# microsoft/GenerativeImage2Text

Hardware: NVIDIA H100
Metric: captions/sec (greedy, max_len=40) GIT_BASE batch64 (higher is better)
Workload: dtype bf16

## Files before the change

generativeimage2text_b200/csrc/attention.cuh:

```cuda
#pragma once
#include "ptx.cuh"
#include "rowops.cuh"

namespace gitb200 {

struct AttnParams {
  const __nv_bfloat16* q;
  const __nv_bfloat16* k;
  const __nv_bfloat16* v;
  __nv_bfloat16* out;
  int B, S, H;
  long long q_rs, kv_rs, q_bs, kv_bs, o_rs, o_bs;
  float scale_log2;
  const int* seq_lens;
};

constexpr int kAttnWgRows = 64;
constexpr int kAttnWgSmem = 5 * 8192 + 64 + 1024;

template <class LoadKV, class Mask>
__device__ __forceinline__ void attn_wg_tile(const CUtensorMap* tmQ, int q_col, int q_row, int nblk, float scale_log2,
                                             const LoadKV& load_kv, const Mask& mask, float (&o)[32]) {
  extern __shared__ __align__(1024) uint8_t attn_smem_raw[];
  uint8_t* smem = attn_smem_raw + ((1024u - (smem_u32(attn_smem_raw) & 1023u)) & 1023u);
// ... 70 lines not shown
    __syncthreads();
    if (tid == 0 && blk + 2 < nblk) issue(blk + 2, st);
  }
#pragma unroll
  for (int i = 0; i < 2; ++i) {
    l_run[i] += __shfl_xor_sync(0xffffffffu, l_run[i], 1);
    l_run[i] += __shfl_xor_sync(0xffffffffu, l_run[i], 2);
  }
  const float inv0 = 1.0f / l_run[0], inv1 = 1.0f / l_run[1];
#pragma unroll
  for (int j = 0; j < 8; ++j) {
    o[4 * j] *= inv0;
    o[4 * j + 1] *= inv0;
    o[4 * j + 2] *= inv1;
    o[4 * j + 3] *= inv1;
  }
}

template <bool kRagged>
__global__ void __launch_bounds__(128) flash_attn_wgmma_kernel(const __grid_constant__ CUtensorMap tmQ,
                                                              const __grid_constant__ CUtensorMap tmK,
                                                              const __grid_constant__ CUtensorMap tmV, const AttnParams p) {
  const int tid = threadIdx.x, warp = tid >> 5, lane = tid & 31;
  const int h = blockIdx.y, b = blockIdx.z;
  const int S = kRagged ? p.seq_lens[b] : p.S;
  const int q0 = blockIdx.x * kAttnWgRows;
  const int row_base = b * p.S;
  if (kRagged && q0 >= S) {
    __nv_bfloat16* og = p.out + b * p.o_bs + h * 64;
    for (int i = tid; i < kAttnWgRows * 8; i += 128) {
      const int r = q0 + (i >> 3);
      if (r < p.S) *reinterpret_cast<uint4*>(og + static_cast<long long>(r) * p.o_rs + (i & 7) * 8) = make_uint4(0, 0, 0, 0);
    }
    return;
  }
  if (tid == 0) {
    tma_prefetch_desc(&tmQ);
    tma_prefetch_desc(&tmK);
    tma_prefetch_desc(&tmV);
  }
  auto load_kv = [&](int blk, uint8_t* sK, uint8_t* sV, uint64_t* bar) {
    tma_load_2d(sK, &tmK, bar, h * 64, row_base + blk * kAttnWgRows);
    tma_load_2d(sV, &tmV, bar, h * 64, row_base + blk * kAttnWgRows);
  };
  auto mask = [&](int blk, float (&s)[32]) {
    const int key0 = blk * kAttnWgRows + 2 * (lane & 3);
#pragma unroll
    for (int j = 0; j < 8; ++j) {
      const int key = key0 + 8 * j;
      if (key >= S) { s[4 * j] = -INFINITY; s[4 * j + 2] = -INFINITY; }
      if (key + 1 >= S) { s[4 * j + 1] = -INFINITY; s[4 * j + 3] = -INFINITY; }
    }
  };
  float o[32];
  attn_wg_tile(&tmQ, h * 64, row_base + q0, (S + kAttnWgRows - 1) / kAttnWgRows, p.scale_log2, load_kv, mask, o);
  const int r0 = q0 + warp * 16 + (lane >> 2), r1 = r0 + 8;
  __nv_bfloat16* og = p.out + b * p.o_bs + h * 64 + 2 * (lane & 3);
#pragma unroll
  for (int j = 0; j < 8; ++j) {
    if (r0 < S) *reinterpret_cast<uint32_t*>(og + static_cast<long long>(r0) * p.o_rs + 8 * j) = pack_bf16(o[4 * j], o[4 * j + 1]);
    else if (kRagged && r0 < p.S) *reinterpret_cast<uint32_t*>(og + static_cast<long long>(r0) * p.o_rs + 8 * j) = 0u;
    if (r1 < S) *reinterpret_cast<uint32_t*>(og + static_cast<long long>(r1) * p.o_rs + 8 * j) = pack_bf16(o[4 * j + 2], o[4 * j + 3]);
// ... 470 lines not shown
      mx = fmaxf(mx, a);
    }
  }
  mx = warp_max(mx);
  float sum = 0.f;
  for (int j = lane; j < n_keys; j += 32) {
    const float e = expf(sc[j] - mx);
    sc[j] = e;
    sum += e;
  }
  sum = warp_sum(sum);
  __syncwarp();
  float a0 = 0.f, a1 = 0.f;
  for (int j = 0; j < n_keys; ++j) {
    const float2 vv = *reinterpret_cast<const float2*>(key_row(j, true) + 2 * lane);
    a0 = fmaf(sc[j], vv.x, a0);
    a1 = fmaf(sc[j], vv.y, a1);
  }
  return make_float2(a0 / sum, a1 / sum);
}

__global__ void __launch_bounds__(128) attn_f32_kernel(const AttnF32Params p) {
  extern __shared__ __align__(16) float attn_f32_smem[];
  const int warp = threadIdx.x >> 5, lane = threadIdx.x & 31;
  float* q_s = attn_f32_smem + warp * (64 + p.S);
  const long long item = static_cast<long long>(blockIdx.x) * 4 + warp;
  const long long total = static_cast<long long>(p.B) * p.H * p.S;
  if (item >= total) return;
  const int row = static_cast<int>(item % p.S);
  const int h = static_cast<int>((item / p.S) % p.H);
  const int b = static_cast<int>(item / (static_cast<long long>(p.S) * p.H));
  const int S = p.seq_lens != nullptr ? p.seq_lens[b] : p.S;
  __nv_bfloat16* orow = p.out + b * p.o_bs + static_cast<long long>(row) * 3 * p.d_model;
  if (row >= S) {
    store_split3_pair(orow, p.d_model, h * 64 + 2 * lane, 0.f, 0.f);
    return;
  }
  const float* qg = p.q + b * p.q_bs + static_cast<long long>(row) * p.q_rs + h * 64;
  q_s[lane] = qg[lane] * 0.125f;
  q_s[lane + 32] = qg[lane + 32] * 0.125f;
  __syncwarp();
  const float2 r = attn_row_f32(q_s, q_s + 64, S, [&](int j, bool want_v) {
    return (want_v ? p.v : p.k) + b * p.kv_bs + static_cast<long long>(j) * p.kv_rs + h * 64;
  });
  store_split3_pair(orow, p.d_model, h * 64 + 2 * lane, r.x, r.y);
}
// ... 99 lines not shown
```

generativeimage2text_b200/csrc/engine_api.inc:

```

extern "C" int gitb200_encode(gitb200_engine* h, const float* images_dev, int batch, int frames, float* feats_out_dev,
                              void* stream) {
  if (!h) return 1;
  const gitb200_engine::NextCall in = take_next_call(h, false);
  ImageBatch ib;
  TRY(image_batch(h, "encode", batch, frames, in.image_hw, &ib));
  if (!images_dev) return fail(h, "encode: null images");
  cudaSetDevice(h->device);
  return encode_impl(h, images_dev, ib, feats_out_dev, static_cast<cudaStream_t>(stream));
}

static int init_src_rows(gitb200_engine* h, cudaStream_t st) {
  const int n = h->cur_rows * h->T_alloc;
  init_src_row_kernel<<<(n + 255) / 256, 256, 0, st>>>(h->src_row[0].as<int>(), h->cur_rows, h->T_alloc);
  CKL(h, "init_src_row_kernel");
  init_src_row_kernel<<<(n + 255) / 256, 256, 0, st>>>(h->src_row[1].as<int>(), h->cur_rows, h->T_alloc);
  CKL(h, "init_src_row_kernel");
  h->cur_src = 0;
  return 0;
}

extern "C" int gitb200_prefill(gitb200_engine* h, int batch, int beam, float* vproj_out_dev, void* stream) {
  if (!h) return 1;
  cudaSetDevice(h->device);
// ... 711 lines not shown
      dst = part_ws.p;
    }
    c = gemm_skinny(static_cast<const bf16*>(a_dev), K, static_cast<const bf16*>(w_dev), K, M, N, K, bias_dev, act, dst, N,
                    out_bf16 != 0, splits, nullptr);
  }
  c.bn = bn;
  int rc = launch_gemm(h, c, st);
  if (rc == 0 && splits > 1) {
    const long long n = static_cast<long long>(M) * N;
    sum_partials_kernel<<<static_cast<int>(std::min<long long>((n + 255) / 256, static_cast<long long>(h->num_sms) * 8)), 256, 0, st>>>(
        part_ws.as<float>(), static_cast<float*>(out_dev), n, c.p.k_splits);
    if (cudaGetLastError() != cudaSuccess) rc = fail(h, "op_gemm: sum_partials_kernel launch failed");
  }
  if (rc != 0) g_create_error = h->err;
  return rc;
}

extern "C" int gitb200_op_layernorm(const float* x_dev, const float* bias_dev, const float* resid_dev,
                                    const float* gamma_dev, const float* beta_dev, float eps, float* out_f32_dev,
                                    void* out_bf16_dev, int rows, int D, void* stream) {
  gitb200_engine* h = op_engine();
  if (!h) return fail(nullptr, "op_layernorm: no CUDA device");
  int rc = launch_ln(h, ln_params(x_dev, bias_dev, resid_dev, gamma_dev, beta_dev, eps, out_f32_dev,
                                  static_cast<bf16*>(out_bf16_dev), rows), D, static_cast<cudaStream_t>(stream));
  if (rc != 0) g_create_error = h->err;
  return rc;
}

static int op_gemm_ex_impl(gitb200_engine* h, const gitb200_gemm_desc& d, int* k_splits_out, cudaStream_t st) {
  if (!d.a || !d.b || !d.out[0]) return fail(h, "op_gemm_ex: null operand or output");
  if (d.M < 1 || d.N < 1 || d.K < 1) return fail(h, "op_gemm_ex: bad shape M=%d N=%d K=%d", d.M, d.N, d.K);
  if (d.act < ACT_NONE || d.act > ACT_QUICKGELU_EXACT) return fail(h, "op_gemm_ex: act %d outside 0 .. 3", d.act);
  if (d.k_splits < 1) return fail(h, "op_gemm_ex: k_splits %d < 1", d.k_splits);
  if (d.split3 && !d.out_bf16) return fail(h, "op_gemm_ex: split3 is a bf16 output format");
  if (d.transposed && (d.resid || d.lse_target || d.seg_n > 0 || d.rows_per_batch > 0))
    return fail(h, "op_gemm_ex: the transposed epilogue has no residual, statistics, column segments or row map");
  if (d.lse_target && (!d.bias || d.resid || d.act || d.out_bf16 || d.seg_n > 0 || d.rows_per_batch > 0 || d.k_splits > 1))
    return fail(h, "op_gemm_ex: the statistics epilogue takes a bias and nothing else");
  if (d.resid && d.ld_resid < d.N) return fail(h, "op_gemm_ex: ld_resid %lld < N", static_cast<long long>(d.ld_resid));
  const int seg_n = d.seg_n > 0 ? d.seg_n : d.N;
  if (d.N % seg_n != 0 || d.N / seg_n > 3) return fail(h, "op_gemm_ex: N=%d is not one to three segments of %d", d.N, seg_n);
  for (int s = 0; s < d.N / seg_n; ++s)
    if (!d.out[s]) return fail(h, "op_gemm_ex: output segment %d is null", s);
  const long long row_elems = d.lse_target ? 2LL * ((d.N + 255) / 256) : (d.transposed ? d.M : seg_n) * (d.split3 ? 3LL : 1LL);
  if (d.ldo < row_elems) return fail(h, "op_gemm_ex: ldo %lld < %lld", static_cast<long long>(d.ldo), row_elems);
  if (d.rows_per_batch > 0 && (d.batch_stride < d.rows_per_batch || d.row_offset < 0 ||
                               d.row_offset + d.rows_per_batch > d.batch_stride))
// ... 15 lines not shown
  return launch_gemm(h, c, st);
}

extern "C" int gitb200_op_gemm_ex(const gitb200_gemm_desc* desc, int* k_splits_out, void* stream) {
  gitb200_engine* h = op_engine();
  if (!h) return fail(nullptr, "op_gemm_ex: no CUDA device");
  const int rc = desc ? op_gemm_ex_impl(h, *desc, k_splits_out, static_cast<cudaStream_t>(stream))
                      : fail(h, "op_gemm_ex: null descriptor");
  if (rc != 0) g_create_error = h->err;
  return rc;
}

static int op_layernorm_ex_impl(gitb200_engine* h, LnParams p, int D, int pre, cudaStream_t st) {
  if (!p.x || !p.gamma || !p.beta) return fail(h, "op_layernorm_ex: null input");
  if (p.rows < 1) return fail(h, "op_layernorm_ex: rows %d < 1", p.rows);
  if (p.n_partials < 1) return fail(h, "op_layernorm_ex: n_partials %d < 1", p.n_partials);
  if (p.n_partials > 1 && p.partial_stride < static_cast<long long>(p.rows) * D)
    return fail(h, "op_layernorm_ex: partial_stride smaller than one partial buffer");
  if (p.split3 && !p.out_bf16) return fail(h, "op_layernorm_ex: split3 is a bf16 output format");
  if (p.remap_F < 0 || (p.remap_F > 0 && (p.remap_B < 1 || p.remap_L < 1 || p.rows != p.remap_B * p.remap_F * p.remap_L)))
    return fail(h, "op_layernorm_ex: %d rows are not B=%d x F=%d x L=%d", p.rows, p.remap_B, p.remap_F, p.remap_L);
  if (p.temb && p.remap_F == 0) return fail(h, "op_layernorm_ex: a temporal embedding needs the frame remap");
  if (pre && D != 768) return fail(h, "op_layernorm_ex: the PRE instantiation exists for D = 768 only");
  return launch_ln(h, p, D, st, pre != 0);
}

extern "C" int gitb200_op_layernorm_ex(const float* x_dev, int n_partials, long long partial_stride, const float* bias_dev,
                                       const float* resid_dev, const float* gamma_dev, const float* beta_dev, float eps,
                                       float* out_f32_dev, void* out_bf16_dev, int rows, int D, int split3,
                                       const float* temb_dev, int remap_B, int remap_F, int remap_L,
                                       const int32_t* skip_flag_dev, int pre, void* stream) {
  gitb200_engine* h = op_engine();
  if (!h) return fail(nullptr, "op_layernorm_ex: no CUDA device");
  LnParams p = ln_params(x_dev, bias_dev, resid_dev, gamma_dev, beta_dev, eps, out_f32_dev, static_cast<bf16*>(out_bf16_dev), rows);
  p.n_partials = n_partials; p.partial_stride = partial_stride;
  p.split3 = split3 ? 1 : 0;
  p.temb = temb_dev; p.remap_B = remap_B; p.remap_F = remap_F; p.remap_L = remap_L;
  p.skip_flag = skip_flag_dev;
  const int rc = op_layernorm_ex_impl(h, p, D, pre, static_cast<cudaStream_t>(stream));
  if (rc != 0) g_create_error = h->err;
  return rc;
}

static int op_lse_combine_impl(gitb200_engine* h, const void* parts, int n_parts, int rows, int T, int V, const int32_t* targets,
                               const int64_t* need_predict, float eps, float* logprob, float* row_loss, int32_t* row_valid,
                               float* loss, cudaStream_t st) {
  if (!parts || !targets || !need_predict || !logprob || !row_loss || !row_valid) return fail(h, "op_lse_combine: null buffer");
// ... 276 lines not shown
```

generativeimage2text_b200/csrc/gemm.cuh:

```cuda
#pragma once
#include "ptx.cuh"

namespace gitb200 {

struct GemmParams {
  int M, N, K;
  int k_splits;
  int transposed;
  int partial;
  long long split_stride;
  int act;
  int out_bf16;
  const float* bias;
  const float* resid;
  long long ld_resid;
  void* out[3];
  long long ldo;
  long long batch_stride;
  int seg_n;
  int rows_per_batch;
  int row_offset;
  const int* skip;
  unsigned long long* dbg;
  int split3;
// ... 245 lines not shown
  const int warp = (threadIdx.x >> 5) & 3;
  const int lane = threadIdx.x & 31;

  if (threadIdx.x == 0) {
    tma_prefetch_desc(&tmA);
    tma_prefetch_desc(&tmB);
    for (int s = 0; s < C::STAGES; ++s) {
      mbar_init(&full[s], 1);
      mbar_init(&empty[s], C::MMA_WGS);
    }
    mbar_fence_init();
  }
  __syncthreads();

  const int m_tiles = (p.M + C::BM - 1) / C::BM;
  const int n_tiles = (p.N + BN - 1) / BN;
  const int kb_total = (p.K + C::BK - 1) / C::BK;
  const int kb_per = (kb_total + p.k_splits - 1) / p.k_splits;
  const int mn_tiles = m_tiles * n_tiles;
  const int num_tiles = mn_tiles * p.k_splits;

  const bool chained = p.chain.counters != nullptr;
  int npre = 0;
  if (kTransposed && p.pdl && static_cast<int>(blockIdx.x) < num_tiles) {
    const int split = static_cast<int>(blockIdx.x) / mn_tiles;
    const int kb0 = split * kb_per;
    npre = min(C::STAGES, min(kb_total, kb0 + kb_per) - kb0);
    if (threadIdx.x == 0) {
      const int m_blk = (static_cast<int>(blockIdx.x) - split * mn_tiles) / n_tiles;
      for (int i = 0; i < npre; ++i) {
        mbar_arrive_expect_tx(&full[i], C::STAGE_BYTES);
        tma_load_2d(sA + i * C::A_BYTES, &tmA, &full[i], (kb0 + i) * C::BK, m_blk * C::BM);
      }
    }
  }
  if (chained) chain_wait(p.chain);
  else if (p.pdl) griddep_wait();
  if (p.pdl) tl_mark(1000 + static_cast<int>(gridDim.x));

  if (wg == 0) {
    setmaxnreg_dec<C::PRODUCER_REGS>();
    if (threadIdx.x == 0) {
      int stage = 0;
      uint32_t phase = 0;
      for (int tile = blockIdx.x; tile < num_tiles; tile += gridDim.x) {
        const int split = tile / mn_tiles;
        const int rem = tile - split * mn_tiles;
        const int m_blk = rem / n_tiles;
        const int n_blk = rem - m_blk * n_tiles;
        const int kb0 = split * kb_per;
        const int kb1 = min(kb_total, kb0 + kb_per);
        for (int kb = kb0; kb < kb1; ++kb) {
          if (npre > 0) {
            --npre;
            tma_load_2d(sB + stage * C::B_BYTES, &tmB, &full[stage], kb * C::BK, n_blk * BN);
          } else {
            mbar_wait(&empty[stage], phase ^ 1);
            mbar_arrive_expect_tx(&full[stage], C::STAGE_BYTES);
            tma_load_2d(sA + stage * C::A_BYTES, &tmA, &full[stage], kb * C::BK, m_blk * C::BM);
            tma_load_2d(sB + stage * C::B_BYTES, &tmB, &full[stage], kb * C::BK, n_blk * BN);
          }
          if (++stage == C::STAGES) {
            stage = 0;
            phase ^= 1;
          }
        }
      }
    }
  } else {
    setmaxnreg_inc<C::MMA_REGS>();
    const int mw = wg - 1;
    const bool store_ok = !(p.pdl && !chained && p.skip != nullptr && *p.skip != 0);
    uint8_t* stg_wg = sStage + mw * C::WG_STAGING_BYTES;
    uint8_t* stg = stg_wg + warp * (32 * 128);
    const int rsub = lane >> 3;
    float acc[BN / 2];
    int stage = 0;
    uint32_t phase = 0;
// ... 108 lines not shown
```

generativeimage2text_b200/csrc/gitb200.cu:

```cuda
#include <cuda.h>
#include <cuda_bf16.h>
#include <cuda_runtime.h>

#include <algorithm>
#include <atomic>
#include <cmath>
#include <cstdarg>
#include <cstdio>
#include <cstring>
#include <map>
#include <mutex>
#include <set>
#include <string>
#include <utility>
#include <vector>

#include "../../include/gitb200.h"
#include "attention.cuh"
#include "constrained.cuh"
#include "decode_mega.cuh"
#include "gemm.cuh"
#include "preproc.cuh"
#include "ptx.cuh"
#include "rowops.cuh"
// ... 376 lines not shown
    case 192: return launch_gemm_bn<192>(h, c, st);
    case 256: return launch_gemm_bn<256>(h, c, st);
    default: return fail(h, "gemm: unsupported tile width %d", bn);
  }
}

static GemmCall gemm_plain(const bf16* A, long long lda, const bf16* W, long long ldw, int M, int N, int K,
                           const float* bias, int act, const float* resid, void* out, bool out_bf16) {
  GemmCall c;
  c.A = A; c.lda = lda; c.B = W; c.ldb = ldw;
  c.p.M = M; c.p.N = N; c.p.K = K; c.p.k_splits = 1;
  c.p.bias = bias; c.p.act = act; c.p.resid = resid; c.p.ld_resid = N;
  c.p.out[0] = out; c.p.ldo = N; c.p.out_bf16 = out_bf16 ? 1 : 0;
  c.p.seg_n = N;
  return c;
}
enum class RowOut { F32, OPERAND, QKV };
static GemmCall gemm_rows(const gitb200_engine* h, RowOut kind, const bf16* A, const bf16* W, int M, int N, int K,
                          const float* bias, int act, const float* resid, void* out) {
  const int ks = h->ks();
  const bool bf16_out = kind == RowOut::OPERAND || (kind == RowOut::QKV && !h->parity);
  GemmCall c = gemm_plain(A, static_cast<long long>(K) * ks, W, static_cast<long long>(K) * ks, M, N, K * ks, bias,
                          (h->parity && act == ACT_QUICKGELU) ? ACT_QUICKGELU_EXACT : act, resid, out, bf16_out);
  if (kind == RowOut::OPERAND && h->parity) {
    c.p.split3 = 1;
    c.p.ldo = 3LL * N;
  }
  return c;
}
static GemmCall gemm_skinny(const bf16* X, long long ldx, const bf16* W, long long ldw, int rows, int feats, int K,
                            const float* bias, int act, void* out, long long ldo, bool out_bf16, int k_splits,
                            const int* skip, bool pdl = false) {
  GemmCall c;
  c.A = W; c.lda = ldw; c.B = X; c.ldb = ldx;
  c.p.M = feats; c.p.N = rows; c.p.K = K; c.p.k_splits = k_splits;
  c.p.transposed = 1; c.p.partial = k_splits > 1 ? 1 : 0;
  c.p.split_stride = static_cast<long long>(rows) * ldo;
  c.p.bias = bias; c.p.act = act;
  c.p.out[0] = out; c.p.ldo = ldo; c.p.out_bf16 = out_bf16 ? 1 : 0;
  c.p.skip = skip;
  c.p.pdl = pdl ? 1 : 0;
  return c;
}

static int launch_ln(gitb200_engine* h, const LnParams& p, int D, cudaStream_t st, bool pdl = false) {
  const int grid = (p.rows + 7) / 8;
  if (D == 768 && pdl) CK(launch_k(true, layernorm_kernel<768, true>, dim3(grid), dim3(256), 0, st, p));
  else if (D == 768) CK(launch_k(false, layernorm_kernel<768, false>, dim3(grid), dim3(256), 0, st, p));
  else if (D == 1024) CK(launch_k(pdl, layernorm_kernel<1024, false>, dim3(grid), dim3(256), 0, st, p));
  else return fail(h, "layernorm: unsupported width %d", D);
  CKL(h, "layernorm_kernel");
  return 0;
}
static LnParams ln_params(const float* x, const float* bias, const float* resid, const float* g, const float* b,
                          float eps, float* of32, bf16* obf16, int rows) {
  LnParams p{};
  p.x = x; p.bias = bias; p.resid = resid; p.gamma = g; p.beta = b; p.eps = eps;
  p.out_f32 = of32; p.out_bf16 = obf16; p.rows = rows;
  return p;
}
static LnParams ln_operand(const gitb200_engine* h, const float* x, const float* g, const float* b, float eps, float* of32,
                           bf16* obf16, int rows) {
  LnParams p = ln_params(x, nullptr, nullptr, g, b, eps, of32, obf16, rows);
  p.split3 = h->parity ? 1 : 0;
  return p;
}

struct SelfAttn {
  const void* q;
  const void* k;
  const void* v;
  bf16* out;
  int B, S, H;
  long long q_rs, kv_rs, q_bs, kv_bs, o_rs, o_bs;
  const int* seq_lens;
};
static int launch_self_attention(gitb200_engine* h, const SelfAttn& a, bool fp32, cudaStream_t st) {
  if (fp32) {
    AttnF32Params p{};
    p.q = static_cast<const float*>(a.q); p.k = static_cast<const float*>(a.k); p.v = static_cast<const float*>(a.v);
    p.out = a.out;
    p.B = a.B; p.S = a.S; p.H = a.H; p.d_model = a.H * 64;
    p.q_rs = a.q_rs; p.kv_rs = a.kv_rs; p.q_bs = a.q_bs; p.kv_bs = a.kv_bs; p.o_bs = a.o_bs;
    p.seq_lens = a.seq_lens;
    const size_t smem = static_cast<size_t>(4) * (64 + p.S) * sizeof(float);
    if (smem > 200 * 1024) return fail(h, "parity attention: %d keys do not fit in shared memory", p.S);
    TRY(set_dyn_smem(h, reinterpret_cast<const void*>(attn_f32_kernel), smem));
    const long long items = static_cast<long long>(p.B) * p.H * p.S;
    attn_f32_kernel<<<static_cast<unsigned int>((items + 3) / 4), 128, smem, st>>>(p);
    CKL(h, "attn_f32_kernel");
    return 0;
  }
  if (a.q_bs != static_cast<long long>(a.S) * a.q_rs || a.kv_bs != static_cast<long long>(a.S) * a.kv_rs)
    return fail(h, "attention: batches must be stored back to back (batch stride = S * row stride)");
  AttnParams p{};
  p.q = static_cast<const bf16*>(a.q); p.k = static_cast<const bf16*>(a.k); p.v = static_cast<const bf16*>(a.v);
  p.out = a.out;
  p.B = a.B; p.S = a.S; p.H = a.H;
  p.q_rs = a.q_rs; p.kv_rs = a.kv_rs; p.q_bs = a.q_bs; p.kv_bs = a.kv_bs; p.o_rs = a.o_rs; p.o_bs = a.o_bs;
  p.scale_log2 = 0.125f * 1.44269504088896340736f;
  p.seq_lens = a.seq_lens;
  const long long rows = static_cast<long long>(a.B) * a.S;
  CUtensorMap tq, tk, tv;
  TRY(get_tmap(h, a.q, rows, a.H * 64, a.q_rs, kAttnWgRows, &tq));
  TRY(get_tmap(h, a.k, rows, a.H * 64, a.kv_rs, kAttnWgRows, &tk));
  TRY(get_tmap(h, a.v, rows, a.H * 64, a.kv_rs, kAttnWgRows, &tv));
  const dim3 grid((a.S + kAttnWgRows - 1) / kAttnWgRows, a.H, a.B);
  if (a.seq_lens != nullptr) flash_attn_wgmma_kernel<true><<<grid, 128, kAttnWgSmem, st>>>(tq, tk, tv, p);
  else flash_attn_wgmma_kernel<false><<<grid, 128, kAttnWgSmem, st>>>(tq, tk, tv, p);
  CKL(h, "flash_attn_wgmma_kernel");
  return 0;
}

struct TextAttn {
  const void* q;
  const void* k;
  const void* v;
  const void* img_k;
  const void* img_v;
  bf16* out;
  int N, T, B, M, H;
  long long o_rs;
  const int* img_lens;
  const int* image_index;
};
static int launch_text_attention(gitb200_engine* h, const TextAttn& a, bool fp32, cudaStream_t st) {
  if (fp32) {
    TextAttnF32Params p{};
    p.q = static_cast<const float*>(a.q); p.k = static_cast<const float*>(a.k); p.v = static_cast<const float*>(a.v);
    p.img_k = static_cast<const float*>(a.img_k); p.img_v = static_cast<const float*>(a.img_v); p.out = a.out;
    p.N = a.N; p.T = a.T; p.H = a.H; p.d_model = a.H * 64; p.M = a.M; p.img_lens = a.img_lens; p.image_index = a.image_index;
    const size_t smem = static_cast<size_t>(4) * (64 + p.M + p.T) * sizeof(float);
// ... 578 lines not shown
  h->cur_img.ragged = false;
  const int B = ib.B, frames = ib.frames, L = ib.L_max;
  TRY(upload_changed(h, h->rg_tab, h->rg_tab_up, ib.imgs.data(), ib.imgs.size() * sizeof(RaggedImg), st));
  if (ib.ragged) TRY(upload_changed(h, h->rg_lens, h->rg_lens_up, ib.lens.data(), ib.lens.size() * sizeof(int), st));
  const int d = h->d, Kp = h->Kp, H = h->cfg.enc_heads;
  const int NI = B * frames;
  const long long Me = static_cast<long long>(NI) * L;
  const int ks = h->ks();
  const bool par = h->parity;
  const size_t qkv_eb = h->kvb();
  CK(h->x.ensure(Me * d * 4));
  CK(h->h.ensure(Me * d * 2 * ks));
  CK(h->qkv.ensure(Me * 3 * d * qkv_eb));
  CK(h->ctx.ensure(Me * d * 2 * ks));
  CK(h->u.ensure(std::max<long long>(Me * 4 * d * 2, static_cast<long long>(NI) * (L - 1) * Kp * 2) * ks));
  CK(h->feats.ensure(Me * d * 2 * ks));
  float* x = h->x.as<float>();
  bf16* hb = h->h.as<bf16>();
  bf16* ctx = h->ctx.as<bf16>();
  bf16* u = h->u.as<bf16>();
  const RaggedImg* tab = h->rg_tab.as<RaggedImg>();
  const float* pos = nullptr;
  TRY(pos_table(h, ib, &pos, st));
  {
    const long long total = static_cast<long long>(NI) * (L - 1) * (Kp / 8);
    const int grid = static_cast<int>(std::min<long long>((total + 255) / 256, h->num_sms * 16));
    im2col_patch_kernel<<<grid, 256, 0, st>>>(images, u, tab, NI, L - 1, h->cfg.patch, Kp, par ? 1 : 0);
    CKL(h, "im2col_patch_kernel");
    GemmCall c = gemm_rows(h, RowOut::F32, u, h->w_patch.as<bf16>(), NI * (L - 1), d, Kp, nullptr, ACT_NONE, nullptr, x);
    c.p.rows_per_batch = L - 1;
    c.p.batch_stride = L;
    c.p.row_offset = 1;
    TRY(launch_gemm(h, c, st));
    const int gridr = static_cast<int>((Me + 7) / 8);
    auto kern = d == 768 ? cls_pos_lnpre_kernel<768> : cls_pos_lnpre_kernel<1024>;
    kern<<<gridr, 256, 0, st>>>(x, h->cls.as<float>(), pos, h->lnpre_g.as<float>(), h->lnpre_b.as<float>(), static_cast<int>(Me), L, tab);
    CKL(h, "cls_pos_lnpre_kernel");
  }
  const int rows = static_cast<int>(Me);
  const char* qkv = h->qkv.as<char>();
  SelfAttn attn{};
  attn.q = qkv; attn.k = qkv + d * qkv_eb; attn.v = qkv + 2 * d * qkv_eb; attn.out = ctx;
  attn.B = NI; attn.S = L; attn.H = H;
  attn.q_rs = attn.kv_rs = 3 * d; attn.q_bs = attn.kv_bs = static_cast<long long>(L) * 3 * d;
  attn.o_rs = d * ks; attn.o_bs = static_cast<long long>(L) * attn.o_rs;
  attn.seq_lens = img_lens(h, ib);
  for (int i = 0; i < h->cfg.enc_layers; ++i) {
    EncLayer& l = h->enc[i];
    TRY(launch_ln(h, ln_operand(h, x, l.ln1g.as<float>(), l.ln1b.as<float>(), 1e-5f, nullptr, hb, rows), d, st));
    TRY(launch_gemm(h, gemm_rows(h, RowOut::QKV, hb, l.wqkv.as<bf16>(), rows, 3 * d, d, l.bqkv.as<float>(), ACT_NONE, nullptr, h->qkv.p), st));
    TRY(launch_self_attention(h, attn, par, st));
    TRY(launch_gemm(h, gemm_rows(h, RowOut::F32, ctx, l.wo.as<bf16>(), rows, d, d, l.bo.as<float>(), ACT_NONE, x, x), st));
    TRY(launch_ln(h, ln_operand(h, x, l.ln2g.as<float>(), l.ln2b.as<float>(), 1e-5f, nullptr, hb, rows), d, st));
    TRY(launch_gemm(h, gemm_rows(h, RowOut::OPERAND, hb, l.w1.as<bf16>(), rows, 4 * d, d, l.b1.as<float>(), ACT_QUICKGELU, nullptr, u), st));
    TRY(launch_gemm(h, gemm_rows(h, RowOut::F32, u, l.w2.as<bf16>(), rows, d, 4 * d, l.b2.as<float>(), ACT_NONE, x, x), st));
  }
  {
    LnParams p = ln_operand(h, x, h->lnpost_g.as<float>(), h->lnpost_b.as<float>(), 1e-5f, feats_out, h->feats.as<bf16>(), rows);
    p.remap_B = B; p.remap_F = frames; p.remap_L = L;
    p.temb = (ib.list_input && h->cfg.num_frames_emb > 0) ? h->temb.as<float>() : nullptr;
    TRY(launch_ln(h, p, d, st));
  }
  h->cur_B = B;
  h->cur_frames = frames;
  h->cur_M = frames * L;
  h->cur_img = ib;
  return 0;
}

constexpr int kQkvSplits = 3, kOutProjSplits = 6, kFc2Splits = 8, kMaxProjSplits = 8;

static char* img_kv_ptr(gitb200_engine* h, int layer, int kv, long long elem_off = 0) {
  const long long per = static_cast<long long>(h->cur_B) * h->cur_M * h->D;
  return h->img_kv.as<char>() + ((static_cast<long long>(layer) * 2 + kv) * per + elem_off) * h->kvb();
}
static char* txt_kv_ptr(gitb200_engine* h, int layer, int kv, long long elem_off = 0) {
  const long long per = static_cast<long long>(h->cur_rows) * h->T_alloc * h->D;
  return h->txt_kv.as<char>() + ((static_cast<long long>(layer) * 2 + kv) * per + elem_off) * h->kvb();
}

static int decoder_buffers(gitb200_engine* h, long long text_rows) {
  const int D = h->D, F = h->F, nl = h->cfg.dec_layers;
  const long long img_rows = static_cast<long long>(h->cur_B) * h->cur_M;
  const long long rows = std::max(img_rows, text_rows);
  const int ks = h->ks();
  const long long kvb = static_cast<long long>(h->kvb());
  CK(h->pt.ensure(rows * D * 4));
  CK(h->pxd.ensure(rows * D * 4));
  CK(h->phd.ensure(rows * D * 2 * ks));
  CK(h->pq.ensure(rows * D * kvb));
  CK(h->pctx.ensure(rows * D * 2 * ks));
  CK(h->pu.ensure(rows * F * 2 * ks));
  CK(h->img_kv.ensure(static_cast<long long>(nl) * 2 * img_rows * D * kvb));
  return 0;
}

template <typename Attend>
static int decoder_layers(gitb200_engine* h, int rows, char* kv, bool kv_per_layer, bool last_qkv_only, Attend&& attend,
                          cudaStream_t st) {
  const int D = h->D, F = h->F, nl = h->cfg.dec_layers;
  const long long kv_bytes = static_cast<long long>(rows) * D * h->kvb();
  float* t = h->pt.as<float>();
  float* xd = h->pxd.as<float>();
  bf16* hd = h->phd.as<bf16>();
  bf16* ctx = h->pctx.as<bf16>();
  bf16* u = h->pu.as<bf16>();
  auto ln = [&](const DevBuf& g, const DevBuf& b) {
    return launch_ln(h, ln_operand(h, t, g.as<float>(), b.as<float>(), 1e-12f, xd, hd, rows), D, st);
  };
  for (int j = 0; j < nl; ++j) {
    DecLayer& l = h->dec[j];
    char* k = kv + (kv_per_layer ? 2 * j * kv_bytes : 0);
    char* v = k + kv_bytes;
    GemmCall c = gemm_rows(h, RowOut::QKV, hd, l.wqkv.as<bf16>(), rows, 3 * D, D, l.bqkv.as<float>(), ACT_NONE, nullptr, h->pq.p);
    c.p.seg_n = D;
    c.p.out[1] = k; c.p.out[2] = v;
    c.p.ldo = D;
    TRY(launch_gemm(h, c, st));
    if (last_qkv_only && j + 1 == nl) break;
    TRY(attend(j, h->pq.p, k, v, ctx));
    TRY(launch_gemm(h, gemm_rows(h, RowOut::F32, ctx, l.wo.as<bf16>(), rows, D, D, l.bo.as<float>(), ACT_NONE, xd, t), st));
    TRY(ln(l.lnag, l.lnab));
    TRY(launch_gemm(h, gemm_rows(h, RowOut::OPERAND, hd, l.w1.as<bf16>(), rows, F, D, l.b1.as<float>(), ACT_GELU_ERF, nullptr, u), st));
    TRY(launch_gemm(h, gemm_rows(h, RowOut::F32, u, l.w2.as<bf16>(), rows, D, F, l.b2.as<float>(), ACT_NONE, xd, t), st));
    TRY(ln(l.lnog, l.lnob));
  }
  return 0;
}

static int image_rows(gitb200_engine* h, float* vproj_out, cudaStream_t st) {
  const int D = h->D, d = h->d, M = h->cur_M, B = h->cur_B;
  const int rows = B * M;
  float* t = h->pt.as<float>();
  float* xd = h->pxd.as<float>();
  TRY(launch_gemm(h, gemm_rows(h, RowOut::F32, h->feats.as<bf16>(), h->w_vp.as<bf16>(), rows, D, d, h->b_vp.as<float>(), ACT_NONE, nullptr, t), st));
  TRY(launch_ln(h, ln_operand(h, t, h->lnvp_g.as<float>(), h->lnvp_b.as<float>(), 1e-5f, xd, h->phd.as<bf16>(), rows), D, st));
  if (vproj_out) CK(cudaMemcpyAsync(vproj_out, xd, static_cast<size_t>(rows) * D * 4, cudaMemcpyDeviceToDevice, st));
  SelfAttn a{};
  a.B = B; a.S = M; a.H = h->cfg.dec_heads;
  a.q_rs = a.kv_rs = D; a.q_bs = a.kv_bs = static_cast<long long>(M) * D;
  a.o_rs = D * h->ks(); a.o_bs = static_cast<long long>(M) * a.o_rs;
  a.seq_lens = img_lens(h, h->cur_img);
  auto self_attention = [&](int, const void* q, const void* k, const void* v, bf16* ctx) {
    a.q = q; a.k = k; a.v = v; a.out = ctx;
    return launch_self_attention(h, a, h->parity, st);
  };
  return decoder_layers(h, rows, h->img_kv.as<char>(), true, true, self_attention, st);
}

static int prefill_impl(gitb200_engine* h, int B, int seqs, int beam, int T_alloc, float* vproj_out, cudaStream_t st) {
  if (B != h->cur_B || h->cur_M <= 0) return fail(h, "prefill: call encode with the same batch first");
  const int D = h->D, F = h->F, nl = h->cfg.dec_layers;
  const int R = B * seqs * beam;
  const int ks = h->ks();
  const long long kvb = static_cast<long long>(h->kvb());
  TRY(decoder_buffers(h, 0));
  {
    const void* before = h->txt_kv.p;
    CK(h->txt_kv.ensure(static_cast<long long>(nl) * 2 * R * T_alloc * D * kvb));
// ... 56 lines not shown
    c.p.chain = cs;
    TRY(launch_gemm(h, c, st));
    next_link(static_cast<unsigned int>(h->last_gemm_grid));
    return 0;
  };
  auto ln_partials = [&](const float* parts, int n, int rows, const float* bias, const float* resid, const float* g,
                         const float* b, float* of32, bf16* obf16) {
    LnParams p = ln_params(parts, bias, resid, g, b, 1e-12f, of32, obf16, rows);
    p.n_partials = n;
    p.partial_stride = static_cast<long long>(rows) * D;
    p.split3 = par ? 1 : 0;
    return p;
  };
  DecodeAttn da{};
  da.n_partials = kQkvSplits;
  da.src_row = src_row; da.ctx = ctx;
  da.B = h->cur_B; da.seqs = h->cur_seqs; da.beam = beam; da.M = h->cur_M; da.T_alloc = h->T_alloc; da.D = D;
  da.state = state;
  da.img_lens = img_lens(h, h->cur_img);
  da.geom = h->attn_geom;
  da.pdl = pdl;
  auto ln = [&](LnParams p) -> int {
    p.skip_flag = skip; p.chain = cs;
    TRY(launch_ln(h, p, D, st, pdl));
    next_link((p.rows + 7) / 8);
    return 0;
  };
  for (int j = 0; j < nl; ++j) {
    DecLayer& l = h->dec[j];
    TRY(skinny(gemm_skinny(hd, D * ks, l.wqkv.as<bf16>(), D * ks, R, 3 * D, D * ks, nullptr, ACT_NONE, qkv, 3 * D, false, kQkvSplits, skip, pdl)));
    da.qkv = qkv; da.bqkv = l.bqkv.as<float>();
    da.img_k = img_kv_ptr(h, j, 0); da.img_v = img_kv_ptr(h, j, 1);
    da.txt_k = txt_kv_ptr(h, j, 0); da.txt_v = txt_kv_ptr(h, j, 1);
    da.chain = cs;
    unsigned int ctas = 0;
    TRY(launch_decode_attention(h, da, par, st, &ctas));
    next_link(ctas);
    TRY(skinny(gemm_skinny(ctx, D * ks, l.wo.as<bf16>(), D * ks, R, D, D * ks, nullptr, ACT_NONE, t, D, false, kOutProjSplits, skip, pdl)));
    TRY(ln(ln_partials(t, kOutProjSplits, R, l.bo.as<float>(), xd, l.lnag.as<float>(), l.lnab.as<float>(), xd, hd)));
    {
      GemmCall c1 = gemm_skinny(hd, D * ks, l.w1.as<bf16>(), D * ks, R, F, D * ks, l.b1.as<float>(), ACT_GELU_ERF, u, static_cast<long long>(F) * ks, true, 1, skip, pdl);
      c1.p.split3 = par ? 1 : 0;
      TRY(skinny(c1));
    }
    TRY(skinny(gemm_skinny(u, F * ks, l.w2.as<bf16>(), F * ks, R, D, F * ks, nullptr, ACT_NONE, t, D, false, kFc2Splits, skip, pdl)));
    TRY(ln(ln_partials(t, kFc2Splits, R, l.b2.as<float>(), xd, l.lnog.as<float>(), l.lnob.as<float>(), xd, hd)));
  }
// ... 17 lines not shown
```

generativeimage2text_b200/csrc/rowops.cuh:

```cuda
#pragma once
#include "ptx.cuh"

namespace gitb200 {

struct StepState {
  int pos;
  int cur_len;
  int finished;
  int final_len;
  int step;
  int empty_caption;
  unsigned int ticket;
  int live;
  int error;
  int bad_draw;
};

enum MegaWaitError : int {
  kWaitGridBarrier = 1,
  kWaitRingFull = 2,
  kWaitRingEmpty = 3,
  kWaitTextKv = 4,
  kWaitRingArmed = 5,
  kWaitTimelineProbe = 99
// ... 188 lines not shown
      for (int a = 0; a < 4; ++a) {
        const int yy = min(max(iy - 1 + a, 0), g0 - 1);
        float4 row = make_float4(0.f, 0.f, 0.f, 0.f);
#pragma unroll
        for (int b = 0; b < 4; ++b) {
          const int xx = min(max(ix - 1 + b, 0), g0 - 1);
          const float4 v = __ldg(src + static_cast<long long>(1 + yy * g0 + xx) * d4 + c);
          row.x += wx[b] * v.x; row.y += wx[b] * v.y; row.z += wx[b] * v.z; row.w += wx[b] * v.w;
        }
        acc.x += wy[a] * row.x; acc.y += wy[a] * row.y; acc.z += wy[a] * row.z; acc.w += wy[a] * row.w;
      }
    }
    reinterpret_cast<float4*>(out)[idx] = acc;
  }
}

struct RaggedImg {
  long long src_off;
  int h, w, gh, gw, L, pos_row;
};

__global__ void im2col_patch_kernel(const float* __restrict__ img, __nv_bfloat16* __restrict__ A,
                                    const RaggedImg* __restrict__ tab, int n_img, int n_slot, int p, int Kp, int split3) {
  const long long total = static_cast<long long>(n_img) * n_slot * (Kp / 8);
  const int K = 3 * p * p;
  for (long long idx = blockIdx.x * static_cast<long long>(blockDim.x) + threadIdx.x; idx < total;
       idx += static_cast<long long>(gridDim.x) * blockDim.x) {
    const int kc = static_cast<int>(idx % (Kp / 8));
    const long long row = idx / (Kp / 8);
    const int im = static_cast<int>(row / n_slot);
    const int t = static_cast<int>(row - static_cast<long long>(im) * n_slot);
    const RaggedImg e = tab[im];
    float v[8];
    if (t < e.gh * e.gw) {
      const int py = t / e.gw, px = t - py * e.gw;
      const float* src = img + e.src_off;
#pragma unroll
      for (int j = 0; j < 8; ++j) {
        const int k = kc * 8 + j;
        float x = 0.f;
        if (k < K) {
          const int c = k / (p * p);
          const int r = k - c * p * p;
          const int ky = r / p;
          const int kx = r - ky * p;
          x = __ldg(src + (static_cast<long long>(c) * e.h + (py * p + ky)) * e.w + (px * p + kx));
// ... 9 lines not shown
      pack_split2(v[0], v[1], hi.x, lo.x);
      pack_split2(v[2], v[3], hi.y, lo.y);
      pack_split2(v[4], v[5], hi.z, lo.z);
      pack_split2(v[6], v[7], hi.w, lo.w);
      uint4* dst = reinterpret_cast<uint4*>(A + row * 3 * Kp) + kc;
      dst[0] = hi; dst[Kp / 8] = lo; dst[Kp / 4] = hi;
      continue;
    }
    uint4 o;
    o.x = pack_bf16(v[0], v[1]);
    o.y = pack_bf16(v[2], v[3]);
    o.z = pack_bf16(v[4], v[5]);
    o.w = pack_bf16(v[6], v[7]);
    reinterpret_cast<uint4*>(A + row * Kp)[kc] = o;
  }
}

template <int D>
__global__ void __launch_bounds__(256)
cls_pos_lnpre_kernel(float* __restrict__ x, const float* __restrict__ cls, const float* __restrict__ pos,
                     const float* __restrict__ gamma, const float* __restrict__ beta, int rows, int L,
                     const RaggedImg* __restrict__ tab) {
  constexpr int NV = D / 128;
  const int row = blockIdx.x * (blockDim.x >> 5) + (threadIdx.x >> 5);
  if (row >= rows) return;
  const int lane = threadIdx.x & 31;
  const int l = row % L;
  const RaggedImg& e = tab[row / L];
  if (l >= e.L) {
    float4* op = reinterpret_cast<float4*>(x + static_cast<long long>(row) * D);
#pragma unroll
    for (int i = 0; i < NV; ++i) op[i * 32 + lane] = make_float4(0.f, 0.f, 0.f, 0.f);
    return;
  }
  pos += static_cast<long long>(e.pos_row) * D;
  float4 v[NV];
  const float4* src = (l == 0) ? reinterpret_cast<const float4*>(cls)
                               : reinterpret_cast<const float4*>(x + static_cast<long long>(row) * D);
  const float4* pp = reinterpret_cast<const float4*>(pos + static_cast<long long>(l) * D);
#pragma unroll
  for (int i = 0; i < NV; ++i) {
    const float4 a = src[i * 32 + lane];
    const float4 b = __ldg(pp + i * 32 + lane);
    v[i] = make_float4(a.x + b.x, a.y + b.y, a.z + b.z, a.w + b.w);
  }
  float mean, rstd;
// ... 413 lines not shown
```

Baseline: 3081.

## Extend programmatic dependent launch to encoder, prefill attention, layernorm and plain GEMMs

Launches the attention kernels, the cls/pos/ln-pre kernel, the layernorms and the plain row GEMMs with programmatic dependent launch. Kernels now trigger early launch and wait on the previous grid, and independent prologue work such as TMA descriptor prefetch runs before the wait. The GEMM prologue can now preload weight tiles before the grid dependency wait in non-transposed mode as well. The pre-instantiation of layernorm is split from the pdl flag. This targets launch gaps between the many small kernels, mainly in encode and prefill. The risk is reading data too early if a weight-only preload assumption does not hold.

```diff
diff --git a/generativeimage2text_b200/csrc/attention.cuh b/generativeimage2text_b200/csrc/attention.cuh
--- a/generativeimage2text_b200/csrc/attention.cuh
+++ b/generativeimage2text_b200/csrc/attention.cuh
@@ -116,6 +116,13 @@
                                                               const __grid_constant__ CUtensorMap tmK,
                                                               const __grid_constant__ CUtensorMap tmV, const AttnParams p) {
   const int tid = threadIdx.x, warp = tid >> 5, lane = tid & 31;
+  griddep_launch_early();
+  if (tid == 0) {
+    tma_prefetch_desc(&tmQ);
+    tma_prefetch_desc(&tmK);
+    tma_prefetch_desc(&tmV);
+  }
+  griddep_wait();
   const int h = blockIdx.y, b = blockIdx.z;
   const int S = kRagged ? p.seq_lens[b] : p.S;
   const int q0 = blockIdx.x * kAttnWgRows;
@@ -127,11 +134,6 @@
       if (r < p.S) *reinterpret_cast<uint4*>(og + static_cast<long long>(r) * p.o_rs + (i & 7) * 8) = make_uint4(0, 0, 0, 0);
     }
     return;
-  }
-  if (tid == 0) {
-    tma_prefetch_desc(&tmQ);
-    tma_prefetch_desc(&tmK);
-    tma_prefetch_desc(&tmV);
   }
   auto load_kv = [&](int blk, uint8_t* sK, uint8_t* sV, uint64_t* bar) {
     tma_load_2d(sK, &tmK, bar, h * 64, row_base + blk * kAttnWgRows);
@@ -648,6 +650,8 @@
 
 __global__ void __launch_bounds__(128) attn_f32_kernel(const AttnF32Params p) {
   extern __shared__ __align__(16) float attn_f32_smem[];
+  griddep_launch_early();
+  griddep_wait();
   const int warp = threadIdx.x >> 5, lane = threadIdx.x & 31;
   float* q_s = attn_f32_smem + warp * (64 + p.S);
   const long long item = static_cast<long long>(blockIdx.x) * 4 + warp;
diff --git a/generativeimage2text_b200/csrc/engine_api.inc b/generativeimage2text_b200/csrc/engine_api.inc
--- a/generativeimage2text_b200/csrc/engine_api.inc
+++ b/generativeimage2text_b200/csrc/engine_api.inc
@@ -757,7 +757,7 @@
   gitb200_engine* h = op_engine();
   if (!h) return fail(nullptr, "op_layernorm: no CUDA device");
   int rc = launch_ln(h, ln_params(x_dev, bias_dev, resid_dev, gamma_dev, beta_dev, eps, out_f32_dev,
-                                  static_cast<bf16*>(out_bf16_dev), rows), D, static_cast<cudaStream_t>(stream));
+                                  static_cast<bf16*>(out_bf16_dev), rows), D, static_cast<cudaStream_t>(stream), false);
   if (rc != 0) g_create_error = h->err;
   return rc;
 }
@@ -819,7 +819,7 @@
     return fail(h, "op_layernorm_ex: %d rows are not B=%d x F=%d x L=%d", p.rows, p.remap_B, p.remap_F, p.remap_L);
   if (p.temb && p.remap_F == 0) return fail(h, "op_layernorm_ex: a temporal embedding needs the frame remap");
   if (pre && D != 768) return fail(h, "op_layernorm_ex: the PRE instantiation exists for D = 768 only");
-  return launch_ln(h, p, D, st, pre != 0);
+  return launch_ln(h, p, D, st, pre != 0, pre != 0);
 }
 
 extern "C" int gitb200_op_layernorm_ex(const float* x_dev, int n_partials, long long partial_stride, const float* bias_dev,
diff --git a/generativeimage2text_b200/csrc/gemm.cuh b/generativeimage2text_b200/csrc/gemm.cuh
--- a/generativeimage2text_b200/csrc/gemm.cuh
+++ b/generativeimage2text_b200/csrc/gemm.cuh
@@ -291,15 +291,18 @@
 
   const bool chained = p.chain.counters != nullptr;
   int npre = 0;
-  if (kTransposed && p.pdl && static_cast<int>(blockIdx.x) < num_tiles) {
+  if (p.pdl && static_cast<int>(blockIdx.x) < num_tiles) {
     const int split = static_cast<int>(blockIdx.x) / mn_tiles;
     const int kb0 = split * kb_per;
     npre = min(C::STAGES, min(kb_total, kb0 + kb_per) - kb0);
     if (threadIdx.x == 0) {
-      const int m_blk = (static_cast<int>(blockIdx.x) - split * mn_tiles) / n_tiles;
+      const int rem = static_cast<int>(blockIdx.x) - split * mn_tiles;
+      const int m_blk = rem / n_tiles;
+      const int n_blk = rem - m_blk * n_tiles;
       for (int i = 0; i < npre; ++i) {
         mbar_arrive_expect_tx(&full[i], C::STAGE_BYTES);
-        tma_load_2d(sA + i * C::A_BYTES, &tmA, &full[i], (kb0 + i) * C::BK, m_blk * C::BM);
+        if (kTransposed) tma_load_2d(sA + i * C::A_BYTES, &tmA, &full[i], (kb0 + i) * C::BK, m_blk * C::BM);
+        else tma_load_2d(sB + i * C::B_BYTES, &tmB, &full[i], (kb0 + i) * C::BK, n_blk * BN);
       }
     }
   }
@@ -322,7 +325,8 @@
         for (int kb = kb0; kb < kb1; ++kb) {
           if (npre > 0) {
             --npre;
-            tma_load_2d(sB + stage * C::B_BYTES, &tmB, &full[stage], kb * C::BK, n_blk * BN);
+            if (kTransposed) tma_load_2d(sB + stage * C::B_BYTES, &tmB, &full[stage], kb * C::BK, n_blk * BN);
+            else tma_load_2d(sA + stage * C::A_BYTES, &tmA, &full[stage], kb * C::BK, m_blk * C::BM);
           } else {
             mbar_wait(&empty[stage], phase ^ 1);
             mbar_arrive_expect_tx(&full[stage], C::STAGE_BYTES);
diff --git a/generativeimage2text_b200/csrc/gitb200.cu b/generativeimage2text_b200/csrc/gitb200.cu
--- a/generativeimage2text_b200/csrc/gitb200.cu
+++ b/generativeimage2text_b200/csrc/gitb200.cu
@@ -422,6 +422,7 @@
   const bool bf16_out = kind == RowOut::OPERAND || (kind == RowOut::QKV && !h->parity);
   GemmCall c = gemm_plain(A, static_cast<long long>(K) * ks, W, static_cast<long long>(K) * ks, M, N, K * ks, bias,
                           (h->parity && act == ACT_QUICKGELU) ? ACT_QUICKGELU_EXACT : act, resid, out, bf16_out);
+  c.p.pdl = h->use_pdl ? 1 : 0;
   if (kind == RowOut::OPERAND && h->parity) {
     c.p.split3 = 1;
     c.p.ldo = 3LL * N;
@@ -443,10 +444,10 @@
   return c;
 }
 
-static int launch_ln(gitb200_engine* h, const LnParams& p, int D, cudaStream_t st, bool pdl = false) {
+static int launch_ln(gitb200_engine* h, const LnParams& p, int D, cudaStream_t st, bool pdl, bool pre = false) {
   const int grid = (p.rows + 7) / 8;
-  if (D == 768 && pdl) CK(launch_k(true, layernorm_kernel<768, true>, dim3(grid), dim3(256), 0, st, p));
-  else if (D == 768) CK(launch_k(false, layernorm_kernel<768, false>, dim3(grid), dim3(256), 0, st, p));
+  if (D == 768 && pre) CK(launch_k(pdl, layernorm_kernel<768, true>, dim3(grid), dim3(256), 0, st, p));
+  else if (D == 768) CK(launch_k(pdl, layernorm_kernel<768, false>, dim3(grid), dim3(256), 0, st, p));
   else if (D == 1024) CK(launch_k(pdl, layernorm_kernel<1024, false>, dim3(grid), dim3(256), 0, st, p));
   else return fail(h, "layernorm: unsupported width %d", D);
   CKL(h, "layernorm_kernel");
@@ -487,7 +488,7 @@
     if (smem > 200 * 1024) return fail(h, "parity attention: %d keys do not fit in shared memory", p.S);
     TRY(set_dyn_smem(h, reinterpret_cast<const void*>(attn_f32_kernel), smem));
     const long long items = static_cast<long long>(p.B) * p.H * p.S;
-    attn_f32_kernel<<<static_cast<unsigned int>((items + 3) / 4), 128, smem, st>>>(p);
+    CK(launch_k(h->use_pdl, attn_f32_kernel, dim3(static_cast<unsigned int>((items + 3) / 4)), dim3(128), smem, st, p));
     CKL(h, "attn_f32_kernel");
     return 0;
   }
@@ -506,8 +507,8 @@
   TRY(get_tmap(h, a.k, rows, a.H * 64, a.kv_rs, kAttnWgRows, &tk));
   TRY(get_tmap(h, a.v, rows, a.H * 64, a.kv_rs, kAttnWgRows, &tv));
   const dim3 grid((a.S + kAttnWgRows - 1) / kAttnWgRows, a.H, a.B);
-  if (a.seq_lens != nullptr) flash_attn_wgmma_kernel<true><<<grid, 128, kAttnWgSmem, st>>>(tq, tk, tv, p);
-  else flash_attn_wgmma_kernel<false><<<grid, 128, kAttnWgSmem, st>>>(tq, tk, tv, p);
+  if (a.seq_lens != nullptr) CK(launch_k(h->use_pdl, flash_attn_wgmma_kernel<true>, grid, dim3(128), kAttnWgSmem, st, tq, tk, tv, p));
+  else CK(launch_k(h->use_pdl, flash_attn_wgmma_kernel<false>, grid, dim3(128), kAttnWgSmem, st, tq, tk, tv, p));
   CKL(h, "flash_attn_wgmma_kernel");
   return 0;
 }
@@ -1132,6 +1133,7 @@
   const RaggedImg* tab = h->rg_tab.as<RaggedImg>();
   const float* pos = nullptr;
   TRY(pos_table(h, ib, &pos, st));
+  const bool pdl = h->use_pdl;
   {
     const long long total = static_cast<long long>(NI) * (L - 1) * (Kp / 8);
     const int grid = static_cast<int>(std::min<long long>((total + 255) / 256, h->num_sms * 16));
@@ -1144,7 +1146,8 @@
     TRY(launch_gemm(h, c, st));
     const int gridr = static_cast<int>((Me + 7) / 8);
     auto kern = d == 768 ? cls_pos_lnpre_kernel<768> : cls_pos_lnpre_kernel<1024>;
-    kern<<<gridr, 256, 0, st>>>(x, h->cls.as<float>(), pos, h->lnpre_g.as<float>(), h->lnpre_b.as<float>(), static_cast<int>(Me), L, tab);
+    CK(launch_k(pdl, kern, dim3(gridr), dim3(256), 0, st, x, h->cls.as<float>(), pos, h->lnpre_g.as<float>(),
+                h->lnpre_b.as<float>(), static_cast<int>(Me), L, tab));
     CKL(h, "cls_pos_lnpre_kernel");
   }
   const int rows = static_cast<int>(Me);
@@ -1157,11 +1160,11 @@
   attn.seq_lens = img_lens(h, ib);
   for (int i = 0; i < h->cfg.enc_layers; ++i) {
     EncLayer& l = h->enc[i];
-    TRY(launch_ln(h, ln_operand(h, x, l.ln1g.as<float>(), l.ln1b.as<float>(), 1e-5f, nullptr, hb, rows), d, st));
+    TRY(launch_ln(h, ln_operand(h, x, l.ln1g.as<float>(), l.ln1b.as<float>(), 1e-5f, nullptr, hb, rows), d, st, pdl));
     TRY(launch_gemm(h, gemm_rows(h, RowOut::QKV, hb, l.wqkv.as<bf16>(), rows, 3 * d, d, l.bqkv.as<float>(), ACT_NONE, nullptr, h->qkv.p), st));
     TRY(launch_self_attention(h, attn, par, st));
     TRY(launch_gemm(h, gemm_rows(h, RowOut::F32, ctx, l.wo.as<bf16>(), rows, d, d, l.bo.as<float>(), ACT_NONE, x, x), st));
-    TRY(launch_ln(h, ln_operand(h, x, l.ln2g.as<float>(), l.ln2b.as<float>(), 1e-5f, nullptr, hb, rows), d, st));
+    TRY(launch_ln(h, ln_operand(h, x, l.ln2g.as<float>(), l.ln2b.as<float>(), 1e-5f, nullptr, hb, rows), d, st, pdl));
     TRY(launch_gemm(h, gemm_rows(h, RowOut::OPERAND, hb, l.w1.as<bf16>(), rows, 4 * d, d, l.b1.as<float>(), ACT_QUICKGELU, nullptr, u), st));
     TRY(launch_gemm(h, gemm_rows(h, RowOut::F32, u, l.w2.as<bf16>(), rows, d, 4 * d, l.b2.as<float>(), ACT_NONE, x, x), st));
   }
@@ -1169,7 +1172,7 @@
     LnParams p = ln_operand(h, x, h->lnpost_g.as<float>(), h->lnpost_b.as<float>(), 1e-5f, feats_out, h->feats.as<bf16>(), rows);
     p.remap_B = B; p.remap_F = frames; p.remap_L = L;
     p.temb = (ib.list_input && h->cfg.num_frames_emb > 0) ? h->temb.as<float>() : nullptr;
-    TRY(launch_ln(h, p, d, st));
+    TRY(launch_ln(h, p, d, st, pdl));
   }
   h->cur_B = B;
   h->cur_frames = frames;
@@ -1216,7 +1219,7 @@
   bf16* ctx = h->pctx.as<bf16>();
   bf16* u = h->pu.as<bf16>();
   auto ln = [&](const DevBuf& g, const DevBuf& b) {
-    return launch_ln(h, ln_operand(h, t, g.as<float>(), b.as<float>(), 1e-12f, xd, hd, rows), D, st);
+    return launch_ln(h, ln_operand(h, t, g.as<float>(), b.as<float>(), 1e-12f, xd, hd, rows), D, st, h->use_pdl);
   };
   for (int j = 0; j < nl; ++j) {
     DecLayer& l = h->dec[j];
@@ -1244,7 +1247,7 @@
   float* t = h->pt.as<float>();
   float* xd = h->pxd.as<float>();
   TRY(launch_gemm(h, gemm_rows(h, RowOut::F32, h->feats.as<bf16>(), h->w_vp.as<bf16>(), rows, D, d, h->b_vp.as<float>(), ACT_NONE, nullptr, t), st));
-  TRY(launch_ln(h, ln_operand(h, t, h->lnvp_g.as<float>(), h->lnvp_b.as<float>(), 1e-5f, xd, h->phd.as<bf16>(), rows), D, st));
+  TRY(launch_ln(h, ln_operand(h, t, h->lnvp_g.as<float>(), h->lnvp_b.as<float>(), 1e-5f, xd, h->phd.as<bf16>(), rows), D, st, h->use_pdl));
   if (vproj_out) CK(cudaMemcpyAsync(vproj_out, xd, static_cast<size_t>(rows) * D * 4, cudaMemcpyDeviceToDevice, st));
   SelfAttn a{};
   a.B = B; a.S = M; a.H = h->cfg.dec_heads;
@@ -1347,7 +1350,7 @@
   da.pdl = pdl;
   auto ln = [&](LnParams p) -> int {
     p.skip_flag = skip; p.chain = cs;
-    TRY(launch_ln(h, p, D, st, pdl));
+    TRY(launch_ln(h, p, D, st, pdl, pdl));
     next_link((p.rows + 7) / 8);
     return 0;
   };
diff --git a/generativeimage2text_b200/csrc/rowops.cuh b/generativeimage2text_b200/csrc/rowops.cuh
--- a/generativeimage2text_b200/csrc/rowops.cuh
+++ b/generativeimage2text_b200/csrc/rowops.cuh
@@ -234,6 +234,7 @@
 
 __global__ void im2col_patch_kernel(const float* __restrict__ img, __nv_bfloat16* __restrict__ A,
                                     const RaggedImg* __restrict__ tab, int n_img, int n_slot, int p, int Kp, int split3) {
+  griddep_launch_early();
   const long long total = static_cast<long long>(n_img) * n_slot * (Kp / 8);
   const int K = 3 * p * p;
   for (long long idx = blockIdx.x * static_cast<long long>(blockDim.x) + threadIdx.x; idx < total;
@@ -289,6 +290,8 @@
                      const float* __restrict__ gamma, const float* __restrict__ beta, int rows, int L,
                      const RaggedImg* __restrict__ tab) {
   constexpr int NV = D / 128;
+  griddep_launch_early();
+  griddep_wait();
   const int row = blockIdx.x * (blockDim.x >> 5) + (threadIdx.x >> 5);
   if (row >= rows) return;
   const int lane = threadIdx.x & 31;
```

After: 3022 (median of 6 runs). -1.9%, worse.
